# ecml-peagnn/graph_recsys_benchmark

Hardware: AMD Instinct MI355X
Metric: BPR-scored edges/sec, PEAGAT MovieLens-25m, emb_dim=64, 9 metapaths (higher is better)
Workload: dtype f32; 1 GPU; ml25m_shaped PEAGAT forward+BPR: N=273744 nodes, 9 metapaths x 2 steps, 208376439 messages/step, emb 64 / hidden 64 / repr 16, batch 4096 triples; headline=True, parallelism=single

## Files before the change

graph_recsys_benchmark_amd/csrc/mlp2.hip:

```cpp
#include "common.h"

namespace pea {
namespace {

typedef float f32x16 __attribute__((ext_vector_type(16)));

__device__ __forceinline__ float4 ld4m(const float *p) { return *reinterpret_cast<const float4 *>(p); }


__host__ __device__ inline int mlp2_image_floats(int ET, int HT) { return HT * ET * 256 + HT * 1024 + 2 * HT * 16; }

__global__ __launch_bounds__(256) void mlp2_pack_kernel(const Mlp2Launch L) {
    const int kPackSplit = (int)gridDim.x / L.n;
    const int chan = (int)blockIdx.x / kPackSplit, part = (int)blockIdx.x % kPackSplit;
    const Mlp2Chan &C = L.c[chan];
    const int EMB = L.emb, HID = L.hid, OUT = L.out;
    const int ET = EMB / 8, HT = HID / 32;
    const int t0 = part * 256 + (int)threadIdx.x, ts = 256 * kPackSplit;
    if (L.kind == PEA_KIND_SAGE) {
        const int KT = 2 * ET;
        float *img = L.images + (size_t)chan * mlp2_image_floats(KT, HT);
        float *wt0 = img, *wt1 = img + HT * KT * 256, *b0p = wt1 + HT * 1024;
        for (int idx = t0; idx < HT * KT * 256; idx += ts) {
            const int e = idx & 3, lane = (idx >> 2) & 63, qq = (idx >> 8) % KT, t = (idx >> 8) / KT;
            const int i = 32 * t + (lane & 31), k = 4 * (2 * (qq % ET) + (lane >> 5)) + e;
            wt0[idx] = (qq < ET ? C.w0 : C.w0_root)[(size_t)i * EMB + k];
        }
        for (int idx = t0; idx < HT * 1024; idx += ts) {
            const int e = idx & 3, lane = (idx >> 2) & 63, g = (idx >> 8) & 3, t = idx >> 10;
            const int j = lane & 31, i = 32 * t + 8 * g + 4 * (lane >> 5) + e;
            wt1[idx] = j < OUT ? C.w1[(size_t)j * HID + i] : j < 2 * OUT ? C.w1_root[(size_t)(j - OUT) * HID + i] : 0.f;
        }
        for (int idx = t0; idx < 2 * HT * 16; idx += ts) {
            const int v = idx & 15, t = (idx >> 4) % HT, half = (idx >> 4) / HT;
            const int i = 32 * t + (v & 3) + 8 * (v >> 2) + 4 * half;
            b0p[idx] = C.b0 ? C.b0[i] : 0.f;
        }
        return;
    }
    float *img = L.images + (size_t)chan * mlp2_image_floats(ET, HT);
    float *wt0 = img, *wt1 = img + HT * ET * 256, *b0p = wt1 + HT * 1024;
    const bool gat = L.kind == PEA_KIND_GAT;
    for (int idx = t0; idx < HT * ET * 256; idx += ts) {
        const int e = idx & 3, lane = (idx >> 2) & 63, q = (idx >> 8) % ET, t = (idx >> 8) / ET;
        const int i = 32 * t + (lane & 31), k = 4 * (2 * q + (lane >> 5)) + e;
        wt0[idx] = gat ? C.w0[(size_t)i * EMB + k] : C.w0[(size_t)k * HID + i];
    }
    for (int idx = t0; idx < HT * 1024; idx += ts) {
        const int e = idx & 3, lane = (idx >> 2) & 63, g = (idx >> 8) & 3, t = idx >> 10;
        const int j = lane & 31, i = 32 * t + 8 * g + 4 * (lane >> 5) + e;
        wt1[idx] = j < OUT ? (gat ? C.w1[(size_t)j * HID + i] : C.w1[(size_t)i * OUT + j]) : 0.f;
    }
    for (int idx = t0; idx < 2 * HT * 16; idx += ts) {
        const int v = idx & 15, t = (idx >> 4) % HT, half = (idx >> 4) / HT;
        const int i = 32 * t + (v & 3) + 8 * (v >> 2) + 4 * half;
        b0p[idx] = C.b0 ? C.b0[i] : 0.f;
    }
    for (int o = t0; o < OUT; o += ts) {
        L.bias1[C.t1_col + o] = C.b1 ? C.b1[o] : 0.f;
        if (gat) {
            L.att_src1[C.t1_col + o] = C.att_src1[o];
            L.att_dst1[C.t1_col + o] = C.att_dst1[o];
        }
    }
    if (gat) {
        for (int k = (int)threadIdx.x * kPackSplit + part; k < EMB; k += ts) {
            float s = 0.f, d = 0.f;
            for (int i = 0; i < HID; ++i) {
                const float w = C.w0[(size_t)i * EMB + k];
                s = fmaf(C.att_src0[i], w, s);
                d = fmaf(C.att_dst0[i], w, d);
            }
            C.ws[k] = s;
            C.wd[k] = d;
        }
    }
}

extern __shared__ float mlp2_lds[];
template <int ET, int HT>
struct Mlp2Cfg {
    static constexpr int kThreads = (ET == 8 && HT == 2) ? 1024 : 512;
};

template <int ET>
struct Mlp2In {
    float4 xa[ET];
    int64_t row;
    bool valid;
};

template <int ET>
__device__ __forceinline__ void mlp2_load(const Mlp2Launch &L, const int *rows, int64_t n_rows, int64_t tile, int ch, int r32,
                                          int half, Mlp2In<ET> &in) {
    const Mlp2Chan &C = L.c[ch];
    const int64_t q0 = tile * 32 + r32;
    in.valid = q0 < n_rows;
    in.row = in.valid ? (rows ? (int64_t)rows[q0] : q0) : 0;
    const bool lone = C.deg0[in.row] != 0;
    const float *src = lone ? L.x + in.row * L.ldx : L.a0 + in.row * L.ld_a0 + C.a0_col;
    float sc = 1.f;
    if (C.dinv && lone) {
        const float di = C.dinv[in.row];
        sc = di * di;
    }
    if (!in.valid) sc = 0.f;
#pragma unroll
    for (int q = 0; q < ET; ++q) {
        const float4 t4 = ld4m(src + 4 * (2 * q + half));
        in.xa[q] = make_float4(sc * t4.x, sc * t4.y, sc * t4.z, sc * t4.w);
    }
}

template <int ET, int HT, bool TRAIN>
__global__ __launch_bounds__((Mlp2Cfg<ET, HT>::kThreads)) void mlp2_kernel(const Mlp2Launch L, const int *__restrict__ rows, int64_t n_rows) {
    constexpr int IMG = HT * ET * 256 + HT * 1024 + 2 * HT * 16;
    const int lane = threadIdx.x & 63, wave = threadIdx.x >> 6, half = lane >> 5, r32 = lane & 31;
    const int64_t n_tiles = (n_rows + 31) / 32;
    constexpr int kMlp2Threads = Mlp2Cfg<ET, HT>::kThreads;
    constexpr int WPB = kMlp2Threads / 64;
    int grp = 0;
    while (grp + 1 < L.n_groups && (int)blockIdx.x >= L.blk_start[grp + 1]) ++grp;
    const int64_t wave_global = (int64_t)((int)blockIdx.x - L.blk_start[grp]) * WPB + wave;
    const int64_t n_waves = (int64_t)(L.blk_start[grp + 1] - L.blk_start[grp]) * WPB;
    {
        const int c0 = grp * L.per_pass;
        const int nc = min(L.per_pass, L.n - c0);
        for (int idx = threadIdx.x * 4; idx < nc * IMG; idx += kMlp2Threads * 4)
            *reinterpret_cast<float4 *>(mlp2_lds + idx) = ld4m(L.images + (size_t)c0 * IMG + idx);
        __syncthreads();
        const int64_t n_items = n_tiles * nc;
        Mlp2In<ET> cur, nxt;
        if (wave_global < n_items) mlp2_load<ET>(L, rows, n_rows, wave_global / nc, c0 + (int)(wave_global % nc), r32, half, cur);
        for (int64_t item = wave_global; item < n_items; item += n_waves) {
            const int cc = (int)(item % nc);
            const int64_t item2 = item + n_waves;
            if (item2 < n_items) mlp2_load<ET>(L, rows, n_rows, item2 / nc, c0 + (int)(item2 % nc), r32, half, nxt);
            const Mlp2Chan &C = L.c[c0 + cc];
            const float *img = mlp2_lds + (size_t)cc * IMG;
            const float *wt0 = img, *wt1 = img + HT * ET * 256, *b0p = wt1 + HT * 1024 + half * HT * 16;
            f32x16 acc[HT];
#pragma unroll
            for (int t = 0; t < HT; ++t)
#pragma unroll
                for (int v = 0; v < 16; ++v) acc[t][v] = 0.f;
#pragma unroll
            for (int q = 0; q < ET; ++q) {
#pragma unroll
                for (int t = 0; t < HT; ++t) {
                    const float4 w = ld4m(wt0 + ((size_t)(t * ET + q) * 64 + lane) * 4);
                    acc[t] = __builtin_amdgcn_mfma_f32_32x32x2f32(w.x, cur.xa[q].x, acc[t], 0, 0, 0);
                    acc[t] = __builtin_amdgcn_mfma_f32_32x32x2f32(w.y, cur.xa[q].y, acc[t], 0, 0, 0);
                    acc[t] = __builtin_amdgcn_mfma_f32_32x32x2f32(w.z, cur.xa[q].z, acc[t], 0, 0, 0);
                    acc[t] = __builtin_amdgcn_mfma_f32_32x32x2f32(w.w, cur.xa[q].w, acc[t], 0, 0, 0);
                }
            }
            f32x16 out;
#pragma unroll
            for (int v = 0; v < 16; ++v) out[v] = 0.f;
            float *hrow = (TRAIN && cur.valid) ? L.h0 + cur.row * L.ld_h0 + C.h0_col + 4 * half : nullptr;
#pragma unroll
            for (int t = 0; t < HT; ++t) {
#pragma unroll
                for (int g = 0; g < 4; ++g) {
                    const float4 w = ld4m(wt1 + ((size_t)(t * 4 + g) * 64 + lane) * 4);
                    const float4 b = ld4m(b0p + t * 16 + 4 * g);
                    const float4 hv = make_float4(fmaxf(acc[t][4 * g + 0] + b.x, 0.f), fmaxf(acc[t][4 * g + 1] + b.y, 0.f),
                                                  fmaxf(acc[t][4 * g + 2] + b.z, 0.f), fmaxf(acc[t][4 * g + 3] + b.w, 0.f));
                    if (TRAIN && hrow) *reinterpret_cast<float4 *>(hrow + 32 * t + 8 * g) = hv;
                    out = __builtin_amdgcn_mfma_f32_32x32x2f32(w.x, hv.x, out, 0, 0, 0);
                    out = __builtin_amdgcn_mfma_f32_32x32x2f32(w.y, hv.y, out, 0, 0, 0);
                    out = __builtin_amdgcn_mfma_f32_32x32x2f32(w.z, hv.z, out, 0, 0, 0);
                    out = __builtin_amdgcn_mfma_f32_32x32x2f32(w.w, hv.w, out, 0, 0, 0);
                }
            }
            if (cur.valid) {
                float *dst = L.t1 + cur.row * L.ld_t1 + C.t1_col;
                const int slot = C.x_slot ? C.x_slot[cur.row] : -1;
                float *dst_x = C.x_buf + (int64_t)(slot < 0 ? 0 : slot) * C.x_ld;
#pragma unroll
                for (int g = 0; g < 4; ++g) {
                    const int j0 = 8 * g + 4 * half;
                    if (j0 < L.out) {
                        const float4 o = make_float4(out[4 * g], out[4 * g + 1], out[4 * g + 2], out[4 * g + 3]);
                        *reinterpret_cast<float4 *>(dst + j0) = o;
                        if (slot >= 0) *reinterpret_cast<float4 *>(dst_x + j0) = o;
                    }
                }
            }
            cur = nxt;
        }
    }
}

template <int ET>
__device__ __forceinline__ void sage_rows(const Mlp2Launch &L, const int *rows, int64_t n_rows, int64_t tile, int r32,
                                          int64_t &row, bool &valid) {
    const int64_t q0 = tile * 32 + r32;
    valid = q0 < n_rows;
    row = valid ? (rows ? (int64_t)rows[q0] : q0) : 0;
}

template <int ET>
__device__ __forceinline__ void sage_load_mean(const Mlp2Launch &L, const Mlp2Chan &C, int64_t row, bool valid, int half,
                                               float4 (&a)[ET]) {
    const bool have = valid && C.deg0[row] == 0;
    const float *src = L.a0 + row * L.ld_a0 + C.a0_col;
#pragma unroll
    for (int q = 0; q < ET; ++q) a[q] = have ? ld4m(src + 4 * (2 * q + half)) : make_float4(0.f, 0.f, 0.f, 0.f);
}

template <int ET, int HT>
__global__ __launch_bounds__(512) void mlp2_sage_kernel(const Mlp2Launch L, const int *__restrict__ rows, int64_t n_rows) {
    constexpr int KT = 2 * ET;
    constexpr int IMG = HT * KT * 256 + HT * 1024 + 2 * HT * 16;
    constexpr int WPB = 512 / 64;
    const int lane = threadIdx.x & 63, wave = threadIdx.x >> 6, half = lane >> 5, r32 = lane & 31;
    const int64_t n_tiles = (n_rows + 31) / 32;
    int grp = 0;
    while (grp + 1 < L.n_groups && (int)blockIdx.x >= L.blk_start[grp + 1]) ++grp;
    const int64_t wave_global = (int64_t)((int)blockIdx.x - L.blk_start[grp]) * WPB + wave;
    const int64_t n_waves = (int64_t)(L.blk_start[grp + 1] - L.blk_start[grp]) * WPB;
    const int c0 = grp * L.per_pass;
    const int nc = min(L.per_pass, L.n - c0);
    for (int idx = threadIdx.x * 4; idx < nc * IMG; idx += 512 * 4)
        *reinterpret_cast<float4 *>(mlp2_lds + idx) = ld4m(L.images + (size_t)c0 * IMG + idx);
    __syncthreads();
    const int64_t n_items = n_tiles * nc;
    float4 a[ET], b[ET];
    int64_t row = 0;
    bool valid = false;
    if (wave_global < n_items) {
        sage_rows<ET>(L, rows, n_rows, wave_global / nc, r32, row, valid);
        sage_load_mean<ET>(L, L.c[c0 + (int)(wave_global % nc)], row, valid, half, a);
    }
    for (int64_t item = wave_global; item < n_items; item += n_waves) {
        const int cc = (int)(item % nc);
        const Mlp2Chan &C = L.c[c0 + cc];
        const float *img = mlp2_lds + (size_t)cc * IMG;
        const float *wt0 = img, *wt1 = img + HT * KT * 256, *b0p = wt1 + HT * 1024 + half * HT * 16;
        {
            const float *src = L.x + row * L.ldx;
#pragma unroll
            for (int q = 0; q < ET; ++q) b[q] = valid ? ld4m(src + 4 * (2 * q + half)) : make_float4(0.f, 0.f, 0.f, 0.f);
        }
        f32x16 acc[HT];
#pragma unroll
        for (int t = 0; t < HT; ++t)
#pragma unroll
            for (int v = 0; v < 16; ++v) acc[t][v] = 0.f;
#pragma unroll
        for (int q = 0; q < ET; ++q) {
#pragma unroll
            for (int t = 0; t < HT; ++t) {
                const float4 w = ld4m(wt0 + ((size_t)(t * KT + q) * 64 + lane) * 4);
                acc[t] = __builtin_amdgcn_mfma_f32_32x32x2f32(w.x, a[q].x, acc[t], 0, 0, 0);
                acc[t] = __builtin_amdgcn_mfma_f32_32x32x2f32(w.y, a[q].y, acc[t], 0, 0, 0);
                acc[t] = __builtin_amdgcn_mfma_f32_32x32x2f32(w.z, a[q].z, acc[t], 0, 0, 0);
                acc[t] = __builtin_amdgcn_mfma_f32_32x32x2f32(w.w, a[q].w, acc[t], 0, 0, 0);
            }
        }
        const int64_t cur_row = row;
        const bool cur_valid = valid;
        const int64_t item2 = item + n_waves;
        if (item2 < n_items) {
            sage_rows<ET>(L, rows, n_rows, item2 / nc, r32, row, valid);
            sage_load_mean<ET>(L, L.c[c0 + (int)(item2 % nc)], row, valid, half, a);
        }
#pragma unroll
        for (int q = 0; q < ET; ++q) {
#pragma unroll
            for (int t = 0; t < HT; ++t) {
                const float4 w = ld4m(wt0 + ((size_t)(t * KT + ET + q) * 64 + lane) * 4);
                acc[t] = __builtin_amdgcn_mfma_f32_32x32x2f32(w.x, b[q].x, acc[t], 0, 0, 0);
                acc[t] = __builtin_amdgcn_mfma_f32_32x32x2f32(w.y, b[q].y, acc[t], 0, 0, 0);
                acc[t] = __builtin_amdgcn_mfma_f32_32x32x2f32(w.z, b[q].z, acc[t], 0, 0, 0);
                acc[t] = __builtin_amdgcn_mfma_f32_32x32x2f32(w.w, b[q].w, acc[t], 0, 0, 0);
            }
        }
        f32x16 out;
#pragma unroll
        for (int v = 0; v < 16; ++v) out[v] = 0.f;
        float *hrow = (L.h0 && cur_valid) ? L.h0 + cur_row * L.ld_h0 + C.h0_col + 4 * half : nullptr;
#pragma unroll
        for (int t = 0; t < HT; ++t) {
#pragma unroll
            for (int g = 0; g < 4; ++g) {
                const float4 w = ld4m(wt1 + ((size_t)(t * 4 + g) * 64 + lane) * 4);
                const float4 bb = ld4m(b0p + t * 16 + 4 * g);
                const float4 hv = make_float4(fmaxf(acc[t][4 * g + 0] + bb.x, 0.f), fmaxf(acc[t][4 * g + 1] + bb.y, 0.f),
                                              fmaxf(acc[t][4 * g + 2] + bb.z, 0.f), fmaxf(acc[t][4 * g + 3] + bb.w, 0.f));
                if (hrow) *reinterpret_cast<float4 *>(hrow + 32 * t + 8 * g) = hv;
                out = __builtin_amdgcn_mfma_f32_32x32x2f32(w.x, hv.x, out, 0, 0, 0);
                out = __builtin_amdgcn_mfma_f32_32x32x2f32(w.y, hv.y, out, 0, 0, 0);
                out = __builtin_amdgcn_mfma_f32_32x32x2f32(w.z, hv.z, out, 0, 0, 0);
                out = __builtin_amdgcn_mfma_f32_32x32x2f32(w.w, hv.w, out, 0, 0, 0);
            }
        }
        if (cur_valid) {
            float *dst_t = L.t1 + cur_row * L.ld_t1 + C.t1_col;
            float *dst_r = L.r1 + cur_row * L.ld_r1 + C.r1_col;
            const int slot = C.x_slot ? C.x_slot[cur_row] : -1;
            float *dst_x = C.x_buf + (int64_t)(slot < 0 ? 0 : slot) * C.x_ld;
#pragma unroll
            for (int g = 0; g < 4; ++g) {
                const int j0 = 8 * g + 4 * half;
                float4 o = make_float4(out[4 * g], out[4 * g + 1], out[4 * g + 2], out[4 * g + 3]);
                if (j0 < L.out) {
                    *reinterpret_cast<float4 *>(dst_t + j0) = o;
                    if (slot >= 0) *reinterpret_cast<float4 *>(dst_x + j0) = o;
                } else if (j0 < 2 * L.out) {
                    const int j = j0 - L.out;
                    if (C.b1) {
                        const float4 b1 = ld4m(C.b1 + j);
                        o = make_float4(o.x + b1.x, o.y + b1.y, o.z + b1.z, o.w + b1.w);
                    }
                    *reinterpret_cast<float4 *>(dst_r + j) = o;
                }
            }
        }
    }
}

}

size_t mlp2_image_bytes(int kind, int emb, int hid) {
    return (size_t)mlp2_image_floats((kind == PEA_KIND_SAGE ? 2 : 1) * emb / 8, hid / 32) * sizeof(float);
}

bool mlp2_supported(int kind, int emb, int hid, int out) {
    return (emb == 64 || emb == 128) && (hid == 64 || hid == 128) && out >= 4 && out % 4 == 0 &&
           out <= (kind == PEA_KIND_SAGE ? 16 : 32);
}

int launch_mlp2_pack(const Mlp2Launch &L, hipStream_t stream) {
    ProfScope ps("pack_weights2", stream);
    const int kt = (L.kind == PEA_KIND_SAGE ? 2 : 1) * L.emb / 8, ht = L.hid / 32;
    const int split = std::max(4, std::min(32, mlp2_image_floats(kt, ht) / 2048));
    PEA_LAUNCH(mlp2_pack_kernel, dim3((unsigned)(L.n * split)), dim3(256), 0, stream, L);
    PEA_HIP(hipGetLastError());
    return PEA_OK;
}

template <int ET, int HT, bool SAGE>
static int launch_mlp2_v(Mlp2Launch L, const int *rows, int64_t n_rows, hipStream_t stream) {
    constexpr size_t img = (size_t)(HT * (SAGE ? 2 * ET : ET) * 256 + HT * 1024 + 2 * HT * 16) * sizeof(float);
    constexpr size_t budget = 160 * 1024 - 2048;
    L.per_pass = (int)std::max<size_t>(1, std::min<size_t>((size_t)L.n, budget / img));
    const int passes = (L.n + L.per_pass - 1) / L.per_pass;
    L.per_pass = (L.n + passes - 1) / passes;
    const size_t lds = (size_t)L.per_pass * img;
    const bool train = !SAGE && L.h0 != nullptr;
    static size_t lds_set_v[2] = {0, 0};
    size_t &lds_set = lds_set_v[train ? 1 : 0];
    const void *fn = SAGE ? reinterpret_cast<const void *>(&mlp2_sage_kernel<ET, HT>)
                          : train ? reinterpret_cast<const void *>(&mlp2_kernel<ET, HT, true>)
                                  : reinterpret_cast<const void *>(&mlp2_kernel<ET, HT, false>);
    if (lds > lds_set) {
        PEA_HIP(hipFuncSetAttribute(fn, hipFuncAttributeMaxDynamicSharedMemorySize, (int)lds));
        lds_set = lds;
    }
    int n_cu = 0;
    PEA_TRY(device_cu_count(&n_cu));
    const int64_t n_tiles = (n_rows + 31) / 32;
    constexpr int kMlp2Threads = SAGE ? 512 : Mlp2Cfg<ET, HT>::kThreads;
    constexpr int WPB = kMlp2Threads / 64;
    L.n_groups = passes;
    int blocks = 0;
    for (int g = 0; g < passes; ++g) {
        const int nc = std::min(L.per_pass, L.n - g * L.per_pass);
        int64_t want = std::max<int64_t>(1, ((int64_t)n_cu * nc + L.n / 2) / L.n);
        want = std::min<int64_t>(want, std::max<int64_t>(1, (n_tiles * nc + WPB - 1) / WPB));
        L.blk_start[g] = blocks;
        blocks += (int)want;
    }
    L.blk_start[passes] = blocks;
    const int grid = blocks;
    ProfScope ps("mlp2_fused", stream, 4.0 * (double)n_rows * (L.emb + (double)L.n * L.out * (SAGE ? 2 : 1)));
    if (SAGE) {
        PEA_REQUIRE(L.h0 == nullptr || L.ld_h0 % 4 == 0, PEA_ERR_ARG, "mlp2: the training variant needs an aligned hidden table");
        PEA_LAUNCH((mlp2_sage_kernel<ET, HT>), dim3((unsigned)grid), dim3(kMlp2Threads), lds, stream, L, rows, n_rows);
    } else if (train) {
        PEA_REQUIRE(L.ld_h0 % 4 == 0, PEA_ERR_ARG, "mlp2: the training variant needs an aligned hidden table");
        PEA_LAUNCH((mlp2_kernel<ET, HT, true>), dim3((unsigned)grid), dim3(kMlp2Threads), lds, stream, L, rows, n_rows);
    } else {
        PEA_LAUNCH((mlp2_kernel<ET, HT, false>), dim3((unsigned)grid), dim3(kMlp2Threads), lds, stream, L, rows, n_rows);
    }
    PEA_HIP(hipGetLastError());
    return PEA_OK;
}

int launch_mlp2(const Mlp2Launch &L, const int *rows, int64_t n_rows, hipStream_t stream) {
    PEA_REQUIRE(mlp2_supported(L.kind, L.emb, L.hid, L.out) && L.n > 0 && L.n <= kMaxMlp2Chan, PEA_ERR_ARG,
                "mlp2: unsupported widths (%d, %d, %d) or %d channels", L.emb, L.hid, L.out, L.n);
    if (n_rows <= 0) return PEA_OK;
    if (L.kind == PEA_KIND_SAGE) {
        PEA_REQUIRE(L.r1 != nullptr, PEA_ERR_ARG, "mlp2: SAGE needs the root-term destination");
        if (L.emb == 64 && L.hid == 64) return launch_mlp2_v<8, 2, true>(L, rows, n_rows, stream);
        if (L.emb == 64 && L.hid == 128) return launch_mlp2_v<8, 4, true>(L, rows, n_rows, stream);
        if (L.emb == 128 && L.hid == 64) return launch_mlp2_v<16, 2, true>(L, rows, n_rows, stream);
        return launch_mlp2_v<16, 4, true>(L, rows, n_rows, stream);
    }
    if (L.emb == 64 && L.hid == 64) return launch_mlp2_v<8, 2, false>(L, rows, n_rows, stream);
    if (L.emb == 64 && L.hid == 128) return launch_mlp2_v<8, 4, false>(L, rows, n_rows, stream);
    if (L.emb == 128 && L.hid == 64) return launch_mlp2_v<16, 2, false>(L, rows, n_rows, stream);
    return launch_mlp2_v<16, 4, false>(L, rows, n_rows, stream);
}

}
```

Measured before the change: 126.2 billion edges/s.

## Switch MLP2 kernel from 32x32x2 to 16x16x4 MFMA with repacked weight images

Rewrites the per-channel two-layer MLP kernel to use 16x16x4 f32 MFMA tiles instead of 32x32x2. Each wave now processes two 16-row halves, and the weight and bias images are repacked to match. The output layer skips its second 16-column tile when out<=16, and input scaling is deferred so the prefetch loads carry no arithmetic. The aim is to cut wasted MFMA work on the 16-wide output, since the 32-wide output tile previously ran half-empty. The cost is more MFMA instructions per item and higher register pressure.

Measured after the change: 129.4 billion edges/s, median of 6. 1.03x the previous value.

```diff
diff --git a/graph_recsys_benchmark_amd/csrc/mlp2.hip b/graph_recsys_benchmark_amd/csrc/mlp2.hip
--- a/graph_recsys_benchmark_amd/csrc/mlp2.hip
+++ b/graph_recsys_benchmark_amd/csrc/mlp2.hip
@@ -4,6 +4,7 @@
 namespace {
 
 typedef float f32x16 __attribute__((ext_vector_type(16)));
+typedef float f32x4 __attribute__((ext_vector_type(4)));
 
 __device__ __forceinline__ float4 ld4m(const float *p) { return *reinterpret_cast<const float4 *>(p); }
 
@@ -41,21 +42,18 @@
     float *img = L.images + (size_t)chan * mlp2_image_floats(ET, HT);
     float *wt0 = img, *wt1 = img + HT * ET * 256, *b0p = wt1 + HT * 1024;
     const bool gat = L.kind == PEA_KIND_GAT;
-    for (int idx = t0; idx < HT * ET * 256; idx += ts) {
-        const int e = idx & 3, lane = (idx >> 2) & 63, q = (idx >> 8) % ET, t = (idx >> 8) / ET;
-        const int i = 32 * t + (lane & 31), k = 4 * (2 * q + (lane >> 5)) + e;
+    const int EJ = EMB / 16, HJ = HID / 16;
+    for (int idx = t0; idx < HJ * EJ * 256; idx += ts) {
+        const int e = idx & 3, lane = (idx >> 2) & 63, j = (idx >> 8) % EJ, t = (idx >> 8) / EJ;
+        const int i = 16 * t + (lane & 15), k = 16 * j + 4 * (lane >> 4) + e;
         wt0[idx] = gat ? C.w0[(size_t)i * EMB + k] : C.w0[(size_t)k * HID + i];
     }
-    for (int idx = t0; idx < HT * 1024; idx += ts) {
-        const int e = idx & 3, lane = (idx >> 2) & 63, g = (idx >> 8) & 3, t = idx >> 10;
-        const int j = lane & 31, i = 32 * t + 8 * g + 4 * (lane >> 5) + e;
-        wt1[idx] = j < OUT ? (gat ? C.w1[(size_t)j * HID + i] : C.w1[(size_t)i * OUT + j]) : 0.f;
-    }
-    for (int idx = t0; idx < 2 * HT * 16; idx += ts) {
-        const int v = idx & 15, t = (idx >> 4) % HT, half = (idx >> 4) / HT;
-        const int i = 32 * t + (v & 3) + 8 * (v >> 2) + 4 * half;
-        b0p[idx] = C.b0 ? C.b0[i] : 0.f;
-    }
+    for (int idx = t0; idx < 2 * HJ * 256; idx += ts) {
+        const int v = idx & 3, lane = (idx >> 2) & 63, t = (idx >> 8) % HJ, u = (idx >> 8) / HJ;
+        const int o = 16 * u + (lane & 15), i = 16 * t + 4 * (lane >> 4) + v;
+        wt1[idx] = o < OUT ? (gat ? C.w1[(size_t)o * HID + i] : C.w1[(size_t)i * OUT + o]) : 0.f;
+    }
+    for (int i = t0; i < HID; i += ts) b0p[i] = C.b0 ? C.b0[i] : 0.f;
     for (int o = t0; o < OUT; o += ts) {
         L.bias1[C.t1_col + o] = C.b1 ? C.b1[o] : 0.f;
         if (gat) {
@@ -85,37 +83,171 @@
 
 template <int ET>
 struct Mlp2In {
-    float4 xa[ET];
-    int64_t row;
-    bool valid;
+    float4 xa[2][ET / 2];
+    float sc[2];
+    int row[2];
+    bool valid[2];
 };
 
 template <int ET>
-__device__ __forceinline__ void mlp2_load(const Mlp2Launch &L, const int *rows, int64_t n_rows, int64_t tile, int ch, int r32,
-                                          int half, Mlp2In<ET> &in) {
+__device__ __forceinline__ void mlp2_load(const Mlp2Launch &L, const int *rows, int64_t n_rows, int64_t tile, int ch, int n16,
+                                          int g, Mlp2In<ET> &in) {
     const Mlp2Chan &C = L.c[ch];
-    const int64_t q0 = tile * 32 + r32;
-    in.valid = q0 < n_rows;
-    in.row = in.valid ? (rows ? (int64_t)rows[q0] : q0) : 0;
-    const bool lone = C.deg0[in.row] != 0;
-    const float *src = lone ? L.x + in.row * L.ldx : L.a0 + in.row * L.ld_a0 + C.a0_col;
-    float sc = 1.f;
-    if (C.dinv && lone) {
-        const float di = C.dinv[in.row];
-        sc = di * di;
-    }
-    if (!in.valid) sc = 0.f;
-#pragma unroll
-    for (int q = 0; q < ET; ++q) {
-        const float4 t4 = ld4m(src + 4 * (2 * q + half));
-        in.xa[q] = make_float4(sc * t4.x, sc * t4.y, sc * t4.z, sc * t4.w);
+    const float *src[2];
+#pragma unroll
+    for (int h = 0; h < 2; ++h) {
+        const int64_t q0 = tile * 32 + 16 * h + n16;
+        in.valid[h] = q0 < n_rows;
+        in.row[h] = in.valid[h] ? (rows ? rows[q0] : (int)q0) : 0;
+    }
+#pragma unroll
+    for (int h = 0; h < 2; ++h) {
+        const bool lone = C.deg0[in.row[h]] != 0;
+        src[h] = (lone ? L.x + (int64_t)in.row[h] * L.ldx : L.a0 + (int64_t)in.row[h] * L.ld_a0 + C.a0_col) + 4 * g;
+        in.sc[h] = 1.f;
+        if (C.dinv) {
+            const float di = C.dinv[in.row[h]];
+            in.sc[h] = lone ? di * di : 1.f;
+        }
+        if (!in.valid[h]) in.sc[h] = 0.f;
+    }
+#pragma unroll
+    for (int h = 0; h < 2; ++h) {
+#pragma unroll
+        for (int j = 0; j < ET / 2; ++j) in.xa[h][j] = ld4m(src[h] + 16 * j);
+    }
+}
+
+template <int ET>
+__device__ __forceinline__ void mlp2_take(Mlp2In<ET> &cur, const Mlp2In<ET> &in) {
+#pragma unroll
+    for (int h = 0; h < 2; ++h) {
+        cur.row[h] = in.row[h];
+        cur.valid[h] = in.valid[h];
+#pragma unroll
+        for (int j = 0; j < ET / 2; ++j) {
+            const float4 t4 = in.xa[h][j];
+            cur.xa[h][j] = make_float4(in.sc[h] * t4.x, in.sc[h] * t4.y, in.sc[h] * t4.z, in.sc[h] * t4.w);
+        }
+    }
+}
+
+template <int ET, int HT, bool TRAIN>
+__device__ __forceinline__ void mlp2_hidden(const Mlp2Launch &L, const Mlp2Chan &C, const float *img, const Mlp2In<ET> &cur, int lane,
+                                            int t0, f32x4 (&acc)[2][4]) {
+    constexpr int EJ = ET / 2;
+    const int g = lane >> 4;
+    const float *wt0 = img, *b0p = img + HT * ET * 256 + HT * 1024;
+#pragma unroll
+    for (int h = 0; h < 2; ++h)
+#pragma unroll
+        for (int t = 0; t < 4; ++t) acc[h][t] = f32x4{0.f, 0.f, 0.f, 0.f};
+#pragma unroll
+    for (int j = 0; j < EJ; ++j) {
+#pragma unroll
+        for (int t = 0; t < 4; ++t) {
+            const float4 w = ld4m(wt0 + ((size_t)((t0 + t) * EJ + j) * 64 + lane) * 4);
+            acc[0][t] = __builtin_amdgcn_mfma_f32_16x16x4f32(w.x, cur.xa[0][j].x, acc[0][t], 0, 0, 0);
+            acc[1][t] = __builtin_amdgcn_mfma_f32_16x16x4f32(w.x, cur.xa[1][j].x, acc[1][t], 0, 0, 0);
+            acc[0][t] = __builtin_amdgcn_mfma_f32_16x16x4f32(w.y, cur.xa[0][j].y, acc[0][t], 0, 0, 0);
+            acc[1][t] = __builtin_amdgcn_mfma_f32_16x16x4f32(w.y, cur.xa[1][j].y, acc[1][t], 0, 0, 0);
+            acc[0][t] = __builtin_amdgcn_mfma_f32_16x16x4f32(w.z, cur.xa[0][j].z, acc[0][t], 0, 0, 0);
+            acc[1][t] = __builtin_amdgcn_mfma_f32_16x16x4f32(w.z, cur.xa[1][j].z, acc[1][t], 0, 0, 0);
+            acc[0][t] = __builtin_amdgcn_mfma_f32_16x16x4f32(w.w, cur.xa[0][j].w, acc[0][t], 0, 0, 0);
+            acc[1][t] = __builtin_amdgcn_mfma_f32_16x16x4f32(w.w, cur.xa[1][j].w, acc[1][t], 0, 0, 0);
+        }
+    }
+#pragma unroll
+    for (int h = 0; h < 2; ++h) {
+        float *hrow = (TRAIN && cur.valid[h]) ? L.h0 + (int64_t)cur.row[h] * L.ld_h0 + C.h0_col + 16 * t0 + 4 * g : nullptr;
+#pragma unroll
+        for (int t = 0; t < 4; ++t) {
+            const float4 b = ld4m(b0p + 16 * (t0 + t) + 4 * g);
+            acc[h][t] = f32x4{fmaxf(acc[h][t][0] + b.x, 0.f), fmaxf(acc[h][t][1] + b.y, 0.f), fmaxf(acc[h][t][2] + b.z, 0.f),
+                              fmaxf(acc[h][t][3] + b.w, 0.f)};
+            if (TRAIN && hrow)
+                *reinterpret_cast<float4 *>(hrow + 16 * t) = make_float4(acc[h][t][0], acc[h][t][1], acc[h][t][2], acc[h][t][3]);
+        }
+    }
+}
+
+__device__ __forceinline__ void mlp2_out_steps(const float *wf, int lane, const f32x4 (&acc)[2][4], f32x4 (&out)[2]) {
+#pragma unroll
+    for (int t = 0; t < 4; ++t) {
+        const float4 w = ld4m(wf + ((size_t)t * 64 + lane) * 4);
+        out[0] = __builtin_amdgcn_mfma_f32_16x16x4f32(w.x, acc[0][t][0], out[0], 0, 0, 0);
+        out[1] = __builtin_amdgcn_mfma_f32_16x16x4f32(w.x, acc[1][t][0], out[1], 0, 0, 0);
+        out[0] = __builtin_amdgcn_mfma_f32_16x16x4f32(w.y, acc[0][t][1], out[0], 0, 0, 0);
+        out[1] = __builtin_amdgcn_mfma_f32_16x16x4f32(w.y, acc[1][t][1], out[1], 0, 0, 0);
+        out[0] = __builtin_amdgcn_mfma_f32_16x16x4f32(w.z, acc[0][t][2], out[0], 0, 0, 0);
+        out[1] = __builtin_amdgcn_mfma_f32_16x16x4f32(w.z, acc[1][t][2], out[1], 0, 0, 0);
+        out[0] = __builtin_amdgcn_mfma_f32_16x16x4f32(w.w, acc[0][t][3], out[0], 0, 0, 0);
+        out[1] = __builtin_amdgcn_mfma_f32_16x16x4f32(w.w, acc[1][t][3], out[1], 0, 0, 0);
+    }
+}
+
+struct Mlp2Dst {
+    float *t1[2], *x[2];
+};
+
+template <int ET>
+__device__ __forceinline__ Mlp2Dst mlp2_dst(const Mlp2Launch &L, const Mlp2Chan &C, const Mlp2In<ET> &cur, int g) {
+    Mlp2Dst d;
+#pragma unroll
+    for (int h = 0; h < 2; ++h) {
+        d.t1[h] = cur.valid[h] ? L.t1 + (int64_t)cur.row[h] * L.ld_t1 + C.t1_col + 4 * g : nullptr;
+        const int slot = (cur.valid[h] && C.x_slot) ? C.x_slot[cur.row[h]] : -1;
+        d.x[h] = slot >= 0 ? C.x_buf + (int64_t)slot * C.x_ld + 4 * g : nullptr;
+    }
+    return d;
+}
+
+__device__ __forceinline__ void mlp2_store_tile(const Mlp2Dst &d, int n_out, int g, int u, const f32x4 (&out)[2]) {
+    if (16 * u + 4 * g >= n_out) return;
+#pragma unroll
+    for (int h = 0; h < 2; ++h) {
+        const float4 o = make_float4(out[h][0], out[h][1], out[h][2], out[h][3]);
+        if (d.t1[h]) *reinterpret_cast<float4 *>(d.t1[h] + 16 * u) = o;
+        if (d.x[h]) *reinterpret_cast<float4 *>(d.x[h] + 16 * u) = o;
+    }
+}
+
+template <int ET, int HT, bool TRAIN>
+__device__ __forceinline__ void mlp2_item(const Mlp2Launch &L, const Mlp2Chan &C, const float *img, const Mlp2In<ET> &cur, int lane,
+                                          bool two_tiles) {
+    constexpr int HJ = 2 * HT;
+    const float *wt1 = img + HT * ET * 256;
+    const int g = lane >> 4;
+    f32x4 acc[2][4];
+    if constexpr (HJ == 4) {
+        mlp2_hidden<ET, HT, TRAIN>(L, C, img, cur, lane, 0, acc);
+        const Mlp2Dst d = mlp2_dst<ET>(L, C, cur, g);
+        const int n_tiles = two_tiles ? 2 : 1;
+        for (int u = 0; u < n_tiles; ++u) {
+            f32x4 out[2] = {f32x4{0.f, 0.f, 0.f, 0.f}, f32x4{0.f, 0.f, 0.f, 0.f}};
+            mlp2_out_steps(wt1 + (size_t)u * HJ * 256, lane, acc, out);
+            mlp2_store_tile(d, L.out, g, u, out);
+        }
+    } else {
+        f32x4 out0[2] = {f32x4{0.f, 0.f, 0.f, 0.f}, f32x4{0.f, 0.f, 0.f, 0.f}};
+        f32x4 out1[2] = {f32x4{0.f, 0.f, 0.f, 0.f}, f32x4{0.f, 0.f, 0.f, 0.f}};
+#pragma unroll
+        for (int t0 = 0; t0 < HJ; t0 += 4) {
+            mlp2_hidden<ET, HT, TRAIN>(L, C, img, cur, lane, t0, acc);
+            mlp2_out_steps(wt1 + (size_t)t0 * 256, lane, acc, out0);
+            if (two_tiles) mlp2_out_steps(wt1 + (size_t)(HJ + t0) * 256, lane, acc, out1);
+        }
+        const Mlp2Dst d = mlp2_dst<ET>(L, C, cur, g);
+        mlp2_store_tile(d, L.out, g, 0, out0);
+        if (two_tiles) mlp2_store_tile(d, L.out, g, 1, out1);
     }
 }
 
 template <int ET, int HT, bool TRAIN>
 __global__ __launch_bounds__((Mlp2Cfg<ET, HT>::kThreads)) void mlp2_kernel(const Mlp2Launch L, const int *__restrict__ rows, int64_t n_rows) {
     constexpr int IMG = HT * ET * 256 + HT * 1024 + 2 * HT * 16;
-    const int lane = threadIdx.x & 63, wave = threadIdx.x >> 6, half = lane >> 5, r32 = lane & 31;
+    const int lane = threadIdx.x & 63, g = lane >> 4, n16 = lane & 15;
+    const int wave = __builtin_amdgcn_readfirstlane(threadIdx.x >> 6);
     const int64_t n_tiles = (n_rows + 31) / 32;
     constexpr int kMlp2Threads = Mlp2Cfg<ET, HT>::kThreads;
     constexpr int WPB = kMlp2Threads / 64;
@@ -130,65 +262,20 @@
             *reinterpret_cast<float4 *>(mlp2_lds + idx) = ld4m(L.images + (size_t)c0 * IMG + idx);
         __syncthreads();
         const int64_t n_items = n_tiles * nc;
+        const bool two_tiles = L.out > 16;
         Mlp2In<ET> cur, nxt;
-        if (wave_global < n_items) mlp2_load<ET>(L, rows, n_rows, wave_global / nc, c0 + (int)(wave_global % nc), r32, half, cur);
+        if (wave_global < n_items) {
+            mlp2_load<ET>(L, rows, n_rows, wave_global / nc, c0 + (int)(wave_global % nc), n16, g, nxt);
+            mlp2_take<ET>(cur, nxt);
+        }
         for (int64_t item = wave_global; item < n_items; item += n_waves) {
             const int cc = (int)(item % nc);
             const int64_t item2 = item + n_waves;
-            if (item2 < n_items) mlp2_load<ET>(L, rows, n_rows, item2 / nc, c0 + (int)(item2 % nc), r32, half, nxt);
+            if (item2 < n_items) mlp2_load<ET>(L, rows, n_rows, item2 / nc, c0 + (int)(item2 % nc), n16, g, nxt);
             const Mlp2Chan &C = L.c[c0 + cc];
             const float *img = mlp2_lds + (size_t)cc * IMG;
-            const float *wt0 = img, *wt1 = img + HT * ET * 256, *b0p = wt1 + HT * 1024 + half * HT * 16;
-            f32x16 acc[HT];
-#pragma unroll
-            for (int t = 0; t < HT; ++t)
-#pragma unroll
-                for (int v = 0; v < 16; ++v) acc[t][v] = 0.f;
-#pragma unroll
-            for (int q = 0; q < ET; ++q) {
-#pragma unroll
-                for (int t = 0; t < HT; ++t) {
-                    const float4 w = ld4m(wt0 + ((size_t)(t * ET + q) * 64 + lane) * 4);
-                    acc[t] = __builtin_amdgcn_mfma_f32_32x32x2f32(w.x, cur.xa[q].x, acc[t], 0, 0, 0);
-                    acc[t] = __builtin_amdgcn_mfma_f32_32x32x2f32(w.y, cur.xa[q].y, acc[t], 0, 0, 0);
-                    acc[t] = __builtin_amdgcn_mfma_f32_32x32x2f32(w.z, cur.xa[q].z, acc[t], 0, 0, 0);
-                    acc[t] = __builtin_amdgcn_mfma_f32_32x32x2f32(w.w, cur.xa[q].w, acc[t], 0, 0, 0);
-                }
-            }
-            f32x16 out;
-#pragma unroll
-            for (int v = 0; v < 16; ++v) out[v] = 0.f;
-            float *hrow = (TRAIN && cur.valid) ? L.h0 + cur.row * L.ld_h0 + C.h0_col + 4 * half : nullptr;
-#pragma unroll
-            for (int t = 0; t < HT; ++t) {
-#pragma unroll
-                for (int g = 0; g < 4; ++g) {
-                    const float4 w = ld4m(wt1 + ((size_t)(t * 4 + g) * 64 + lane) * 4);
-                    const float4 b = ld4m(b0p + t * 16 + 4 * g);
-                    const float4 hv = make_float4(fmaxf(acc[t][4 * g + 0] + b.x, 0.f), fmaxf(acc[t][4 * g + 1] + b.y, 0.f),
-                                                  fmaxf(acc[t][4 * g + 2] + b.z, 0.f), fmaxf(acc[t][4 * g + 3] + b.w, 0.f));
-                    if (TRAIN && hrow) *reinterpret_cast<float4 *>(hrow + 32 * t + 8 * g) = hv;
-                    out = __builtin_amdgcn_mfma_f32_32x32x2f32(w.x, hv.x, out, 0, 0, 0);
-                    out = __builtin_amdgcn_mfma_f32_32x32x2f32(w.y, hv.y, out, 0, 0, 0);
-                    out = __builtin_amdgcn_mfma_f32_32x32x2f32(w.z, hv.z, out, 0, 0, 0);
-                    out = __builtin_amdgcn_mfma_f32_32x32x2f32(w.w, hv.w, out, 0, 0, 0);
-                }
-            }
-            if (cur.valid) {
-                float *dst = L.t1 + cur.row * L.ld_t1 + C.t1_col;
-                const int slot = C.x_slot ? C.x_slot[cur.row] : -1;
-                float *dst_x = C.x_buf + (int64_t)(slot < 0 ? 0 : slot) * C.x_ld;
-#pragma unroll
-                for (int g = 0; g < 4; ++g) {
-                    const int j0 = 8 * g + 4 * half;
-                    if (j0 < L.out) {
-                        const float4 o = make_float4(out[4 * g], out[4 * g + 1], out[4 * g + 2], out[4 * g + 3]);
-                        *reinterpret_cast<float4 *>(dst + j0) = o;
-                        if (slot >= 0) *reinterpret_cast<float4 *>(dst_x + j0) = o;
-                    }
-                }
-            }
-            cur = nxt;
+            mlp2_item<ET, HT, TRAIN>(L, C, img, cur, lane, two_tiles);
+            mlp2_take<ET>(cur, nxt);
         }
     }
 }
```
